# parsakhaz/multimodal-image-similarity-search

Hardware: AMD Instinct MI355X
Metric: images/s CLIP-B/32 encode @ bs256; Mvec/s cosine top-10 over 10M x 512 (higher is better)
Workload: dtype bf16

## Files before the change

### multimodal-image-similarity-search_amd/csrc/api_index.hip

```cpp
#include "common.h"
#include <queue>
#include "retrieval_kernels.h"
#include "gemm_bf16_256.h"
#include "gemm_bf16_p256.h"
#include <algorithm>

struct mmiss_index {
    int dim = 0, dtype = MMISS_F32, device = 0, elt = 4;
    int qelt() const { return dtype == MMISS_F32 ? 4 : 2; }
    hipStream_t own_stream = nullptr, user_stream = nullptr;
    bool has_user_stream = false;
    hipEvent_t done_ev = nullptr;
    bool async_pending = false;
    std::mutex mu;
    int64_t count = 0, capacity = 0;
    DevBuf rows, labels_d;
    DevBuf inv;
    std::vector<int64_t> labels_h;
    DevBuf tags;
    std::vector<uint64_t> tags_h;
    DevBuf fmask, fmask2, tag_stage;
    DevBuf stage, qn, qs, qstage, lists_s, lists_r, lists2_s, lists2_r, cand, cur_s, cur_r, out_c, map, gmax;
    DevBuf qmap, qmap64, qs2, cand2;
    DevBuf eps_q, thr, thr2, swp_cnt, swp_list;
// ... 511 lines not shown
    MM_NO_PENDING(ix, "mmiss_index_get_tags");
    std::vector<int64_t> lab;
    MM_TRY(fetch_i64(labels, n, lab));
    std::vector<uint64_t> val((size_t)n);
    for (int64_t i = 0; i < n; ++i) {
        const int64_t r = find_row(ix, lab[i]);
        if (r < 0) MM_FAIL(MMISS_ERR_ARG, "mmiss_index_get_tags: label %lld not in the index", (long long)lab[i]);
        val[i] = ix->tags_h[(size_t)r];
    }
    if (mmiss_is_device_ptr(out)) {
        MM_TRY(mmiss_use_device(ix->device));
        MM_HIP(hipMemcpyAsync(out, val.data(), (size_t)n * 8, hipMemcpyHostToDevice, ix->stream()));
        MM_HIP(hipStreamSynchronize(ix->stream()));
    } else {
        memcpy(out, val.data(), (size_t)n * 8);
    }
    return MMISS_OK;
}

namespace {

constexpr int SWEEP_CAP = 8192;

void guard_terms(const mmiss_index* ix, double* fixed, double* cnorm) {
    const double D = ix->dim;
    const double cn = ix->dtype == MMISS_F8 ? 1.07 : 1.0 + ldexp(1.0, -9);
    double e = 4.0 * D * ldexp(1.0, -24) * cn * (1.0 + ldexp(1.0, -9));
    if (ix->dtype != MMISS_F32) e += D * ldexp(1.0, -25) * cn;
    if (ix->dtype == MMISS_F8) e += ldexp(1.0, -23);
    *fixed = e * 1.003 + ldexp(1.0, -21);
    *cnorm = ix->dtype == MMISS_F32 ? 0.0 : cn * 1.003;
}

int launch_rerank(mmiss_index* ix, hipStream_t st, const RerankArgs& r, int blocks) {
    int npow = 1;
    while (npow < r.ncand) npow <<= 1;
    const int lds = npow * 8 + 16;
    MM_PROF("rerank", st, 2.0 * blocks * r.ncand * r.D, (double)blocks * r.ncand * r.D * ix->elt);
    const int threads = r.ncand >= 16 ? 1024 : 256;
    void (*kern)(RerankArgs) = with_storage(ix->dtype, [](auto s) { return &rerank_kernel<typename decltype(s)::T>; });
    if (lds > 32768) MM_TRY(mmiss_ensure_dyn_lds(reinterpret_cast<const void*>(kern), lds));
    hipLaunchKernelGGL(kern, dim3(blocks), dim3(threads), lds, st, r);
    MM_HIP(hipGetLastError());
    return MMISS_OK;
}

int exhaustive_queries(mmiss_index* ix, hipStream_t st, const mmiss_index::Pending& pd, const std::vector<int32_t>& which) {
    const int64_t N = ix->count;
    const int D = ix->dim, KP = 32;
    const int kk = (int)std::min<int64_t>(pd.k, N);
    const int kkpad = (int)round_up(std::max(kk, 1), KP);
    const int nq = (int)which.size();
    if (nq == 0 || N <= 0) return MMISS_OK;
    MM_TRY(ix->dist_all.ensure((size_t)N * 4));
    MM_TRY(ix->dist_pin.ensure((size_t)N * 4, st));
    const float* dist = ix->dist_pin.as<float>();
    std::vector<int32_t> cand((size_t)nq * kkpad, -1);
    typedef std::pair<float, int32_t> Ent;
    for (int i = 0; i < nq; ++i) {
        const int32_t q = which[i];
        {
            MM_PROF("canonical_scan", st, 2.0 * N * D, (double)N * D * ix->elt);
            const int grid = (int)std::min<int64_t>(8192, (N + 15) / 16);
            with_storage(ix->dtype, [&](auto s) {
                hipLaunchKernelGGL(canonical_scan_kernel<typename decltype(s)::T>, dim3(grid), dim3(256), 0, st, ix->rows.p, N, D,
                                   ix->qn.as<float>() + (size_t)q * D, ix->dist_all.as<float>(), (const float*)ix->inv.as<float>());
            });
// ... 265 lines not shown
    MM_TRY(ix->eps_q.ensure((size_t)Qpad * 4));
    MM_TRY(ix->thr.ensure((size_t)Qpad * 4));
    MM_PROF("prep_queries", st, 4.0 * Q * D, (double)Q * D * (8 + ix->elt));
    double eps_fixed, cnorm;
    guard_terms(ix, &eps_fixed, &cnorm);
    with_storage(ix->dtype, [&](auto s) {
        using QT = typename decltype(s)::Q;
        hipLaunchKernelGGL(prep_queries_kernel<QT>, dim3((Qpad + 3) / 4), dim3(256), 0, st, qsrc, ix->qn.as<float>(), ix->qs.as<QT>(),
                           Q, Qpad, D, ix->eps_q.as<float>(), eps_fixed, cnorm);
    });
    MM_HIP(hipGetLastError());
    return MMISS_OK;
}

int dense_pass(mmiss_index* ix, hipStream_t st, const QueryPlan& p, int Q) {
    const int D = ix->dim, kp = p.kp;
    const int64_t N = ix->count;
    const int ng = (int)(p.Ndense / 16);
    MM_TRY(ix->gmax.ensure((size_t)p.Mq * ng * 4));
    GemmEpi ep{};
    ep.out = ix->gmax.p; ep.ldo = ng; ep.m_valid = Q; ep.p0 = (int)N; ep.m_fast = 1;
    ep.aux = ix->inv.as<float>();
    {
        MM_PROF(p.dense8 ? (p.sample ? "score_gemm_f8_sample" : "score_gemm_f8") : (p.sample ? "score_gemm_f16_sample" : "score_gemm_f16"), st,
                2.0 * Q * (double)std::min<int64_t>(N, p.Ndense) * D, (double)std::min<int64_t>(N, p.Ndense) * D * ix->elt);
        if (p.big) MM_TRY(launch_strip_gemm(ix, st, p.strip_v3, ix->qs.p, ep, p.Mq, (int)p.Ndense, p.strip, nullptr));
        else MM_TRY((launch_gemm_inst<_Float16, 128, MMISS_EPI_GROUPMAX_F32>(st, ix->qs.p, ix->rows.p, ep, p.Mq, (int)p.Npad, D)));
    }
    const int units = (ng + 1023) / 1024;
    int splits = (1024 + Q - 1) / Q;
    if (splits > units) splits = units;
    if (splits > 32) splits = 32;
    if (splits < 1) splits = 1;
    MM_TRY(ix->lists_s.ensure((size_t)splits * Q * kp * 4));
    MM_TRY(ix->lists_r.ensure((size_t)splits * Q * kp * 4));
    SelectArgs sa{};
    sa.G = ix->gmax.as<float>(); sa.ldg = ng; sa.ng = ng; sa.kp = kp; sa.Q = Q;
    sa.out_s = ix->lists_s.as<float>(); sa.out_r = ix->lists_r.as<int32_t>();
    {
        MM_PROF("select_topk", st, 0.0, (double)Q * ng * 4);
        hipLaunchKernelGGL(select_topk_kernel, dim3(Q, splits), dim3(256), 0, st, sa);
        MM_HIP(hipGetLastError());
    }
    MergeArgs m{};
    m.in_s = ix->lists_s.as<float>(); m.in_r = ix->lists_r.as<int32_t>();
    m.L = splits; m.Q = Q; m.kp = kp;
    if (p.sample) {
        const int cap = p.filter_cap;
        MM_TRY(ix->seed_s.ensure((size_t)p.Mq * kp * 4));
        MM_TRY(ix->seed_r.ensure((size_t)p.Mq * kp * 4));
        MM_TRY(ix->fcnt.ensure((size_t)p.Mq * 4));
        MM_TRY(ix->fbuf_s.ensure((size_t)p.Mq * cap * 4));
        MM_TRY(ix->fbuf_g.ensure((size_t)p.Mq * cap * 4));
        {
            MergeArgs m1 = m;
            m1.lists_per_block = splits; m1.out_s = ix->seed_s.as<float>(); m1.out_r = ix->seed_r.as<int32_t>();
            MM_PROF("merge_lists", st, 0.0, (double)splits * Q * kp * 8);
            hipLaunchKernelGGL(merge_lists_kernel, dim3(Q, 1), dim3(256), 0, st, m1);
            MM_HIP(hipGetLastError());
        }
        MM_HIP(hipMemsetAsync(ix->fcnt.p, 0, (size_t)p.Mq * 4, st));
        StripFilter flt{};
        flt.tau = ix->seed_s.as<float>() + (kp - 1); flt.tau_stride = kp;
        flt.cnt = ix->fcnt.as<int32_t>(); flt.buf_s = ix->fbuf_s.as<float>(); flt.buf_g = ix->fbuf_g.as<int32_t>();
        flt.cap = cap; flt.bn_begin = (int)p.ns_tiles;
        {
            MM_PROF(p.dense8 ? "score_gemm_f8" : "score_gemm_f16", st, 2.0 * Q * (double)(N - p.Ndense) * D, (double)(N - p.Ndense) * D * ix->elt);
            MM_TRY(launch_strip_gemm(ix, st, p.strip_v3, ix->qs.p, ep, p.Mq, (int)p.Npad, p.strip, &flt));
        }
        m.in_s = ix->seed_s.as<float>(); m.in_r = ix->seed_r.as<int32_t>(); m.L = 1;
        m.flat_s = ix->fbuf_s.as<float>(); m.flat_r = ix->fbuf_g.as<int32_t>(); m.flat_cnt = ix->fcnt.as<int32_t>();
        m.flat_cap = cap;
    }
    m.cand = ix->cand.as<int32_t>(); m.cand_stride = p.ncand; m.page_off = 0;
    m.cur_s = ix->cur_s.as<float>(); m.cur_r = ix->cur_r.as<int32_t>();
    return launch_merge(ix, st, m);
}

int scan_pass(mmiss_index* ix, hipStream_t st, const QueryPlan& qp, int Q) {
    const mmiss_index::Pending& pd = ix->pend;
    const int kp = qp.kp;
    const ScanPlan p = plan_scan(ix->dim, ix->qelt(), Q, kp, ix->count);
    MM_TRY(ix->lists_s.ensure((size_t)p.slabs * Q * kp * 4));
    MM_TRY(ix->lists_r.ensure((size_t)p.slabs * Q * kp * 4));
    const bool paging = qp.pages > 1;
    if (paging) {
        std::vector<float> inf((size_t)Q, INFINITY);
        std::vector<int32_t> neg((size_t)Q, -1);
        MM_HIP(hipMemcpyAsync(ix->cur_s.p, inf.data(), (size_t)Q * 4, hipMemcpyHostToDevice, st));
        MM_HIP(hipMemcpyAsync(ix->cur_r.p, neg.data(), (size_t)Q * 4, hipMemcpyHostToDevice, st));
        MM_HIP(hipStreamSynchronize(st));
    }
    for (int page = 0; page < qp.pages; ++page) {
        ScanArgs a{};
        a.rows = ix->rows.p; a.N = ix->count; a.D = ix->dim; a.inv = ix->inv.as<float>(); a.qs = ix->qs.p; a.Q = Q;
        a.cur_s = paging ? ix->cur_s.as<float>() : nullptr;
        a.cur_r = paging ? ix->cur_r.as<int32_t>() : nullptr;
        a.kp = kp; a.tiles_per_block = p.tiles_per_block;
        a.out_s = ix->lists_s.as<float>(); a.out_r = ix->lists_r.as<int32_t>();
        if (pd.filt) { a.tags = ix->tags.as<uint64_t>(); a.req = pd.d_mask; a.exc = pd.d_mask + Q; }
        MM_TRY(launch_scan(ix, st, a, p));
        MergeArgs m{};
        m.in_s = ix->lists_s.as<float>(); m.in_r = ix->lists_r.as<int32_t>();
        m.L = p.slabs; m.Q = Q; m.kp = kp;
        m.cand = ix->cand.as<int32_t>(); m.cand_stride = qp.ncand; m.page_off = page * kp;
        m.cur_s = ix->cur_s.as<float>(); m.cur_r = ix->cur_r.as<int32_t>();
        MM_TRY(launch_merge(ix, st, m));
    }
// ... 332 lines not shown
```

### multimodal-image-similarity-search_amd/csrc/retrieval_kernels.h

```cpp
#pragma once
#include "common.h"
#include "gemm_bf16.h"
#include <math.h>
#include <type_traits>

#define SCAN_NEG_INF (-INFINITY)
#define SCAN_ROW_NONE 0x7fffffff

__device__ __forceinline__ double wave_butterfly_sum(double v) {
#pragma unroll
    for (int o = 32; o > 0; o >>= 1) v = v + __shfl_xor(v, o);
    return v;
}

#define MMISS_F8_SCALE 128.0f
struct F8 {
    uint8_t b;
    F8() = default;
    __device__ explicit F8(float y) { b = (uint8_t)(__builtin_amdgcn_cvt_pk_fp8_f32(y * MMISS_F8_SCALE, 0.0f, 0, false) & 0xff); }
    __device__ explicit operator float() const { return __builtin_amdgcn_cvt_f32_fp8((int)b, 0) * (1.0f / MMISS_F8_SCALE); }
};
__device__ __forceinline__ void f8x4_values(uint32_t w, float (&v)[4]) {
    v[0] = __builtin_amdgcn_cvt_f32_fp8((int)w, 0) * (1.0f / MMISS_F8_SCALE);
    v[1] = __builtin_amdgcn_cvt_f32_fp8((int)w, 1) * (1.0f / MMISS_F8_SCALE);
// ... 442 lines not shown
            if (lane >= 32 && lane - 32 < cw) {
                s = cs_all[(w * NQ + ql) * CAP + lane - 32];
                r = cr_all[(w * NQ + ql) * CAP + lane - 32];
            }
            wave_sort64(s, r, lane);
        }
        if (lane < a.kp) {
            const size_t o = ((size_t)blockIdx.x * a.Q + q) * a.kp + lane;
            a.out_s[o] = s;
            a.out_r[o] = (r == SCAN_ROW_NONE) ? -1 : r;
        }
    }
}

struct SelectArgs {
    const float* G;
    int ldg;
    int ng;
    int kp;
    float* out_s;
    int32_t* out_r;
    int Q;
};

__device__ __forceinline__ void lane_list_insert(float& ls, int& lr, float xs, int xr, int lane) {
    const unsigned long long better = __ballot(ls > xs || (ls == xs && lr < xr));
    const int p = __popcll(better);
    const float us = __int_as_float(__builtin_amdgcn_update_dpp(__float_as_int(ls), __float_as_int(ls), 0x138, 0xF, 0xF, false));
    const int ur = __builtin_amdgcn_update_dpp(lr, lr, 0x138, 0xF, 0xF, false);
    if (lane > p) { ls = us; lr = ur; }
    else if (lane == p) { ls = xs; lr = xr; }
}

__global__ __launch_bounds__(256) void select_topk_kernel(SelectArgs a) {
    __shared__ float ms[4][32];
    __shared__ int mr[4][32];
    const int tid = threadIdx.x, lane = tid & 63, wave = tid >> 6;
    const int q = blockIdx.x;
    const int nsplit = gridDim.y;
    const int units = (a.ng + 1023) / 1024;
    const int upb = (units + nsplit - 1) / nsplit;
    const int c_begin = blockIdx.y * upb * 1024;
    int c_end = c_begin + upb * 1024;
    if (c_end > a.ng) c_end = a.ng;
    const float* row = a.G + (size_t)q * a.ldg;

    float ls = SCAN_NEG_INF;
    int lr = SCAN_ROW_NONE;
    float tau = SCAN_NEG_INF;
    int tau_r = SCAN_ROW_NONE;
    auto fetch = [&](int c0) {
        const int c = c0 + lane * 4;
        f32x4 v = {SCAN_NEG_INF, SCAN_NEG_INF, SCAN_NEG_INF, SCAN_NEG_INF};
        if (c0 >= c_end) return v;
        if (c + 3 < c_end) {
            v = *reinterpret_cast<const f32x4*>(row + c);
        } else {
#pragma unroll
            for (int e = 0; e < 4; ++e)
                if (c + e < c_end) v[e] = row[c + e];
        }
        return v;
    };
    f32x4 vnext = fetch(c_begin + wave * 256);
    for (int c0 = c_begin + wave * 256; c0 < c_end; c0 += 1024) {
        const int c = c0 + lane * 4;
        const f32x4 v = vnext;
        vnext = fetch(c0 + 1024);
        const bool seed = (c0 == c_begin + wave * 256);
        if (seed) {
            ls = v[0];
            lr = (c < c_end) ? c : SCAN_ROW_NONE;
            wave_sort64(ls, lr, lane);
            tau = __shfl(ls, a.kp - 1);
            tau_r = __shfl(lr, a.kp - 1);
        }
#pragma unroll
        for (int e = 0; e < 4; ++e) {
            if (seed && e == 0) continue;
            const float s = v[e];
            unsigned long long m = __ballot(s > tau || (s == tau && c + e < tau_r));
            while (m) {
                const int src = __ffsll((long long)m) - 1;
                m &= m - 1;
                const float xs = __shfl(s, src);
                const int xr = c0 + src * 4 + e;
                if (!(xs > tau || (xs == tau && xr < tau_r))) continue;
                lane_list_insert(ls, lr, xs, xr, lane);
                tau = __shfl(ls, a.kp - 1);
                tau_r = __shfl(lr, a.kp - 1);
            }
        }
    }
    if (lane < 32) { ms[wave][lane] = ls; mr[wave][lane] = lr; }
    __syncthreads();
    if (wave == 0) {
        float s = (lane < 32) ? ms[0][lane] : ms[1][lane - 32];
        int r = (lane < 32) ? mr[0][lane] : mr[1][lane - 32];
        wave_sort64(s, r, lane);
        for (int w = 2; w < 4; ++w) {
            if (lane >= 32) { s = ms[w][lane - 32]; r = mr[w][lane - 32]; }
            wave_sort64(s, r, lane);
        }
        if (lane < a.kp) {
            const size_t o = ((size_t)blockIdx.y * a.Q + q) * a.kp + lane;
            a.out_s[o] = s;
            a.out_r[o] = (r == SCAN_ROW_NONE) ? -1 : r;
        }
    }
}

struct MergeArgs {
    const float* in_s;
    const int32_t* in_r;
    int L, Q, kp;
    int32_t* cand;
    int cand_stride, page_off;
    float* cur_s;
    int32_t* cur_r;
    int lists_per_block;
    float* out_s;
    int32_t* out_r;
    const float* flat_s;
    const int32_t* flat_r;
    const int32_t* flat_cnt;
    int flat_cap;
};

__global__ __launch_bounds__(256) void merge_lists_kernel(MergeArgs a) {
    __shared__ float cs[4][64];
    __shared__ int cr[4][64];
    __shared__ int cnt[4];
    const int tid = threadIdx.x, lane = tid & 63, wave = tid >> 6;
    const int q = blockIdx.x;
    const int kp = a.kp;
    if (lane == 0) cnt[wave] = 0;
    __builtin_amdgcn_fence(__ATOMIC_SEQ_CST, "wavefront");
    float tau = SCAN_NEG_INF;
    const int l_begin = a.out_s ? blockIdx.y * a.lists_per_block : 0;
    int l_end = a.out_s ? l_begin + a.lists_per_block : a.L;
    if (l_end > a.L) l_end = a.L;
    const int64_t list_total = (int64_t)(l_end > l_begin ? l_end - l_begin : 0) * kp;
    int64_t total = list_total;
    if (a.flat_s) {
        const int c = a.flat_cnt[q];
        total += c < a.flat_cap ? c : a.flat_cap;
    }
    const int NL = 64 - kp;
    auto fetch = [&](int64_t e0, float& s, int& r) {
        s = SCAN_NEG_INF;
        r = -1;
        const int64_t e = e0 + lane;
        if (lane < NL && e < total) {
            if (e < list_total) {
                const int64_t l = l_begin + e / kp;
                const int slot = (int)(e % kp);
                const size_t o = ((size_t)l * a.Q + q) * kp + slot;
                s = a.in_s[o];
                r = a.in_r[o];
            } else {
                const size_t o = (size_t)q * a.flat_cap + (size_t)(e - list_total);
                s = a.flat_s[o];
                r = a.flat_r[o];
            }
        }
    };
    float s, sn;
    int r, rn;
    int64_t e0 = (int64_t)wave * NL;
    fetch(e0, s, r);
    while (e0 < total) {
        const int64_t e1 = e0 + 4 * (int64_t)NL;
        fetch(e1, sn, rn);
        if (r >= 0 && s > tau) {
            const int pos = atomicAdd(&cnt[wave], 1);
            cs[wave][pos] = s;
            cr[wave][pos] = r;
        }
        __builtin_amdgcn_fence(__ATOMIC_SEQ_CST, "wavefront");
        const int c = cnt[wave];
        if (c > kp) {
            float ss = SCAN_NEG_INF;
            int rr = SCAN_ROW_NONE;
            if (lane < c) { ss = cs[wave][lane]; rr = cr[wave][lane]; }
            wave_sort64(ss, rr, lane);
            if (lane < kp) { cs[wave][lane] = ss; cr[wave][lane] = rr; }
            tau = __shfl(ss, kp - 1);
            if (lane == 0) cnt[wave] = kp;
            __builtin_amdgcn_fence(__ATOMIC_SEQ_CST, "wavefront");
        }
        e0 = e1;
        s = sn;
// ... 4 lines not shown
        float s = SCAN_NEG_INF;
        int r = SCAN_ROW_NONE;
        const int c0 = cnt[0];
        if (lane < c0) { s = cs[0][lane]; r = cr[0][lane]; }
        wave_sort64(s, r, lane);
        for (int w = 1; w < 4; ++w) {
            const int cw = cnt[w];
            if (cw == 0) continue;
            if (lane >= kp) { s = SCAN_NEG_INF; r = SCAN_ROW_NONE; }
            if (lane >= 32 && lane - 32 < cw) { s = cs[w][lane - 32]; r = cr[w][lane - 32]; }
            wave_sort64(s, r, lane);
        }
        const bool valid = lane < kp && r != SCAN_ROW_NONE;
        if (a.out_s) {
            if (lane < kp) {
                const size_t o = ((size_t)blockIdx.y * a.Q + q) * kp + lane;
                a.out_s[o] = valid ? s : SCAN_NEG_INF;
                a.out_r[o] = valid ? r : -1;
            }
            return;
        }
        if (lane < kp) a.cand[(size_t)q * a.cand_stride + a.page_off + lane] = valid ? r : -1;
        if (a.cur_s) {
            const unsigned long long m = __ballot(valid);
            const int nvalid = __popcll(m);
            const float ls = __shfl(s, nvalid > 0 ? nvalid - 1 : 0);
            const int lr = __shfl(r, nvalid > 0 ? nvalid - 1 : 0);
            if (lane == 0) {
                if (nvalid == kp) { a.cur_s[q] = ls; a.cur_r[q] = lr; }
                else { a.cur_s[q] = SCAN_NEG_INF; a.cur_r[q] = SCAN_ROW_NONE; }
            }
        }
    }
}

struct RerankArgs {
    const void* rows; int D;
    const float* qn;
    const int32_t* cand;
    int cand_stride, ncand;
    int group_mode;
    int64_t nrows;
    const int64_t* labels;
    int k;
    int64_t* out_labels;
    float* out_dist;
    int32_t* out_count;
    const int32_t* qmap;
    int32_t* out_rows;
    const float* tau;
    double eps;
    int32_t* flags;
    int32_t* nflag;
    int force_flag;
    const int32_t* ovf_cnt;
    int ovf_cap;
    const float* eps_q;
    float* thr_out;
    const int32_t* cand_cnt;
    const int32_t* bmap;
    const float* inv;
    int32_t* cnt_host;
};

template <typename T>
__device__ __forceinline__ void canon_partial_dots(const T* rv, bool live, const float* qp, int D, double (&acc)[4]) {
    acc[0] = acc[1] = acc[2] = acc[3] = 0.0;
    typedef typename std::conditional<sizeof(T) == 1, uint32_t, typename std::conditional<sizeof(T) == 2, u32x2, f32x4>::type>::type piece_t;
    for (int d0 = 0; d0 < D; d0 += 512) {
        piece_t w[8];
        f32x4 qq[8];
#pragma unroll
        for (int u = 0; u < 8; ++u) {
            w[u] = piece_t{};
            qq[u] = f32x4{0.f, 0.f, 0.f, 0.f};
            if (d0 + 64 * u < D) {
                qq[u] = *reinterpret_cast<const f32x4*>(qp + d0 + 64 * u);
                if (live) w[u] = *reinterpret_cast<const piece_t*>(rv + d0 + 64 * u);
            }
        }
#pragma unroll
        for (int u = 0; u < 8; ++u) {
            if (d0 + 64 * u < D) {
                float rr[4];
                if constexpr (sizeof(T) == 1) {
                    f8x4_values(w[u], rr);
                } else if constexpr (sizeof(T) == 2) {
                    const _Float16* h = reinterpret_cast<const _Float16*>(&w[u]);
#pragma unroll
                    for (int j = 0; j < 4; ++j) rr[j] = (float)h[j];
                } else {
#pragma unroll
                    for (int j = 0; j < 4; ++j) rr[j] = w[u][j];
                }
#pragma unroll
                for (int j = 0; j < 4; ++j) acc[j] = acc[j] + (double)qq[u][j] * (double)rr[j];
            }
        }
    }
}

template <typename T>
__global__ __launch_bounds__(1024) void rerank_kernel(RerankArgs a) {
    extern __shared__ __attribute__((aligned(16))) char smem[];
    const int tid = threadIdx.x, lane = tid & 63, wave = tid >> 6;
    const int b = blockIdx.x;
    const int q = a.qmap ? a.qmap[b] : b;
    const int lb = a.bmap ? a.bmap[b] : b;
    int nc = a.ncand;
    if (a.cand_cnt) {
        const int cc = a.cand_cnt[lb];
        if (a.cnt_host && tid == 0) a.cnt_host[b] = cc;
        nc = cc < nc ? cc : nc;
    }
    int npow = 1;
    while (npow < nc) npow <<= 1;
    float* sd = reinterpret_cast<float*>(smem);
    int32_t* sr = reinterpret_cast<int32_t*>(smem + (size_t)npow * 4);
    const float* qv = a.qn + (size_t)q * a.D;
    const int nthreads = blockDim.x, nwaves = blockDim.x >> 6;
    for (int i = tid; i < npow; i += nthreads) { sd[i] = INFINITY; sr[i] = INT32_MAX; }
    __syncthreads();
    const int p16 = lane & 15, sub = lane >> 4;
    for (int c0 = wave * 4; c0 < nc; c0 += nwaves * 4) {
        const int c = c0 + sub;
        int64_t row = -1;
        if (c < nc) {
            if (a.group_mode) {
                const int g = a.cand[(size_t)lb * a.cand_stride + (c >> 4)];
                if (g >= 0) {
                    row = groupmax_row(g, c & 15);
                    if (row >= a.nrows) row = -1;
                }
            } else {
                row = a.cand[(size_t)lb * a.cand_stride + c];
            }
        }
        const bool live = row >= 0;
        const T* rv = reinterpret_cast<const T*>(a.rows) + (size_t)(live ? row : 0) * a.D + 4 * p16;
        const float* qp = qv + 4 * p16;
        double acc[4];
        canon_partial_dots<T>(rv, live, qp, a.D, acc);
#pragma unroll
        for (int o = 8; o > 0; o >>= 1) {
#pragma unroll
            for (int j = 0; j < 4; ++j) acc[j] = acc[j] + __shfl_xor(acc[j], o);
        }
        const double t0 = acc[0] + acc[2], t1 = acc[1] + acc[3];
        double dot = t0 + t1;
        if (p16 == 0 && row >= 0) {
            if constexpr (sizeof(T) == 1) dot = dot * (double)a.inv[row];
            sd[c] = (float)(1.0 - dot);
            sr[c] = (int32_t)row;
        }
    }
    __syncthreads();
    for (int k = 2; k <= npow; k <<= 1) {
        for (int j = k >> 1; j > 0; j >>= 1) {
            for (int i = tid; i < npow; i += nthreads) {
                const int p = i ^ j;
                if (p > i) {
                    const float di = sd[i], dp = sd[p];
                    const int32_t li = sr[i], lp = sr[p];
                    const bool up = (i & k) == 0;
                    const bool i_first = (di < dp) || (di == dp && li < lp) || (dp != dp && di == di);
                    const bool p_first = (dp < di) || (dp == di && lp < li) || (di != di && dp == dp);
                    const bool swap = up ? p_first : i_first;
                    if (swap) { sd[i] = dp; sd[p] = di; sr[i] = lp; sr[p] = li; }
                }
            }
            __syncthreads();
        }
    }
    for (int i = tid; i < a.k; i += nthreads) {
        const bool ok = i < npow && sr[i] != INT32_MAX;
        a.out_labels[(size_t)q * a.k + i] = ok ? a.labels[sr[i]] : -1;
        a.out_dist[(size_t)q * a.k + i] = ok ? sd[i] : INFINITY;
    }
    const int64_t k_eff = (int64_t)a.k < a.nrows ? (int64_t)a.k : a.nrows;
    if (a.out_rows) {
        for (int i = tid; i < a.cand_stride && i < (int)((k_eff + 31) & ~31LL); i += nthreads)
            a.out_rows[(size_t)b * a.cand_stride + i] = (i < k_eff && i < npow && sr[i] != INT32_MAX) ? sr[i] : -1;
    }
    if (tid == 0) {
        int nvalid = 0;
        const int lim = a.k < npow ? a.k : npow;
        for (int i = 0; i < lim; ++i) nvalid += (sr[i] != INT32_MAX);
        a.out_count[q] = nvalid;
        const double eps = a.eps_q ? (double)a.eps_q[q] : a.eps;
        if (a.flags) {
            int flag = 0;
            const float t = a.tau ? a.tau[b] : SCAN_NEG_INF;
            if (t > SCAN_NEG_INF) {
                if (nvalid < k_eff || a.force_flag) flag = 1;
                else if (a.ovf_cnt && a.ovf_cnt[q] > a.ovf_cap) flag = 1;
                else {
                    const double ck = 1.0 - (double)sd[k_eff - 1];
                    if (!(ck - (double)t > eps)) flag = 1;
                }
            }
            a.flags[b] = flag;
            if (flag && a.nflag) atomicAdd(a.nflag, 1);
        }
        if (a.thr_out) {
            float thr = SCAN_NEG_INF;
            if (k_eff > 0 && nvalid >= k_eff) {
                const double lim = (1.0 - (double)sd[k_eff - 1]) - eps;
                thr = (float)lim;
                if ((double)thr > lim) thr = nextafterf(thr, -INFINITY);
                if (!(lim == lim)) thr = SCAN_NEG_INF;
            }
            a.thr_out[q] = thr;
        }
    }
}

template <typename T>
__global__ __launch_bounds__(256) void canonical_scan_kernel(const void* __restrict__ rows, int64_t N, int D,
                                                             const float* __restrict__ qv, float* __restrict__ dist,
                                                             const float* __restrict__ inv) {
    const int lane = threadIdx.x & 63, wave = threadIdx.x >> 6;
    const int p16 = lane & 15, sub = lane >> 4;
    const float* qp = qv + 4 * p16;
    for (int64_t r0 = ((int64_t)blockIdx.x * 4 + wave) * 4; r0 < N; r0 += (int64_t)gridDim.x * 16) {
        const int64_t row = r0 + sub;
        const bool live = row < N;
        const T* rv = reinterpret_cast<const T*>(rows) + (size_t)(live ? row : 0) * D + 4 * p16;
        double acc[4];
        canon_partial_dots<T>(rv, live, qp, D, acc);
#pragma unroll
        for (int o = 8; o > 0; o >>= 1) {
#pragma unroll
            for (int j = 0; j < 4; ++j) acc[j] = acc[j] + __shfl_xor(acc[j], o);
        }
        const double t0 = acc[0] + acc[2], t1 = acc[1] + acc[3];
        double dot = t0 + t1;
        if (p16 == 0 && live) {
            if constexpr (sizeof(T) == 1) dot = dot * (double)inv[row];
            dist[row] = (float)(1.0 - dot);
        }
// ... 132 lines not shown
```

### multimodal-image-similarity-search_amd/csrc/encoder_kernels.h

```cpp
#pragma once
#include "common.h"
#include "attention_stream.h"

template <bool SRC_U8>
__global__ __launch_bounds__(256) void im2col_kernel(const void* __restrict__ pixels, uint16_t* __restrict__ out,
                                                     int B, int S, int P, int Kp) {
    const int G = S / P;
    const int PP = P * P;
    const int Kreal = 3 * PP;
    const int kgroups = Kp >> 3;
    const int64_t total = (int64_t)B * G * G * kgroups;
    const float mean[3] = {0.48145466f, 0.4578275f, 0.40821073f};
    const float istd[3] = {1.0f / 0.26862954f, 1.0f / 0.26130258f, 1.0f / 0.27577711f};
    for (int64_t idx = (int64_t)blockIdx.x * blockDim.x + threadIdx.x; idx < total;
         idx += (int64_t)gridDim.x * blockDim.x) {
        const int kg = (int)(idx % kgroups);
        const int64_t m = idx / kgroups;
        const int b = (int)(m / (G * G));
        const int pr = (int)(m - (int64_t)b * G * G);
        const int py = pr / G, px = pr - py * G;
        const int k0 = kg << 3;
        float v[8];
        if (!SRC_U8 && (P & 7) == 0 && k0 < Kreal) {
            const int c = k0 / PP, rem = k0 - c * PP, ky = rem / P, kx = rem - ky * P;
            const float* src = reinterpret_cast<const float*>(pixels) +
                               (((size_t)b * 3 + c) * S + (size_t)py * P + ky) * S + (size_t)px * P + kx;
            const f32x4 a = *reinterpret_cast<const f32x4*>(src);
            const f32x4 d = *reinterpret_cast<const f32x4*>(src + 4);
            v[0] = a[0]; v[1] = a[1]; v[2] = a[2]; v[3] = a[3];
            v[4] = d[0]; v[5] = d[1]; v[6] = d[2]; v[7] = d[3];
        } else {
#pragma unroll
            for (int e = 0; e < 8; ++e) {
                const int k = k0 + e;
                float x = 0.f;
// ... 964 lines not shown
        case 6: return heads(std::integral_constant<int, 6>{});
    }
    const int lds = NKP * 32 * (128 + ATT_VSTRIDE);
    const int rounds = ((T + 15) / 16 + 3) / 4;
    int qs = 256 / (B * H);
    qs = qs < 1 ? 1 : (qs > rounds ? rounds : qs);
    MM_TRY(mmiss_ensure_dyn_lds(reinterpret_cast<const void*>(&attention_kernel<NKP, false, true>), lds));
    hipLaunchKernelGGL((attention_kernel<NKP, false, true>), dim3(B * H, qs), dim3(256), lds, st, (const uint16_t*)qkv, (uint16_t*)nullptr, T, H,
                       ctx8, ctxs, ld_s);
    MM_HIP(hipGetLastError());
    return MMISS_OK;
}
static int launch_attention_mx_short(hipStream_t st, const void* qkv, uint8_t* ctx8, uint8_t* ctxs, int ld_s, int B, int T, int H) {
    int hpb = mmiss_option("att_hpb", 0);
    if (hpb == 0) {
        hpb = 1;
        for (int c : {4, 6, 3, 2})
            if (H % c == 0 && (int64_t)B * (H / c) >= 512) { hpb = c; break; }
    }
    if (!((hpb == 2 || hpb == 3 || hpb == 4 || hpb == 6) && H % hpb == 0)) hpb = 1;
    switch ((T + 31) / 32) {
        case 1: return launch_attention_mx_nkp<1>(st, hpb, qkv, ctx8, ctxs, ld_s, B, T, H);
        case 2: return launch_attention_mx_nkp<2>(st, hpb, qkv, ctx8, ctxs, ld_s, B, T, H);
        case 3: return launch_attention_mx_nkp<3>(st, hpb, qkv, ctx8, ctxs, ld_s, B, T, H);
        default: return launch_attention_mx_nkp<4>(st, hpb, qkv, ctx8, ctxs, ld_s, B, T, H);
    }
}

static int launch_attention(hipStream_t st, const void* qkv, void* ctx, int B, int T, int H, bool causal) {
    if (B <= 0) return MMISS_OK;
    if (T <= 0 || T > 288 || H <= 0) MM_FAIL(MMISS_ERR_UNSUPPORTED, "attention: T=%d (1..288), H=%d", T, H);
    const int nkp = (T + 31) / 32;
    MM_PROF("attention", st, 4.0 * B * H * (double)T * T * 64, (double)B * T * H * 64 * 2 * 4);
    if (nkp <= 4) {
        int hpb = mmiss_option("att_hpb", 0);
        if (hpb == 0) {
            hpb = 1;
            for (int c : {4, 6, 3, 2})
                if (H % c == 0 && (int64_t)B * (H / c) >= 512) { hpb = c; break; }
        }
        if ((hpb == 2 || hpb == 3 || hpb == 4 || hpb == 6) && H % hpb == 0) {
            switch (nkp) {
                case 1: return launch_attention_heads_hpb<1>(st, hpb, qkv, ctx, B, T, H, causal);
                case 2: return launch_attention_heads_hpb<2>(st, hpb, qkv, ctx, B, T, H, causal);
                case 3: return launch_attention_heads_hpb<3>(st, hpb, qkv, ctx, B, T, H, causal);
                default: return launch_attention_heads_hpb<4>(st, hpb, qkv, ctx, B, T, H, causal);
            }
        }
    }
    switch (nkp) {
        case 1: return launch_attention_nkp<1>(st, qkv, ctx, B, T, H, causal);
        case 2: return launch_attention_nkp<2>(st, qkv, ctx, B, T, H, causal);
        case 3: return launch_attention_nkp<3>(st, qkv, ctx, B, T, H, causal);
        case 4: return launch_attention_nkp<4>(st, qkv, ctx, B, T, H, causal);
    }
    return causal ? launch_attention_long<true, false>(st, qkv, ctx, nullptr, nullptr, 0, B, T, H)
                  : launch_attention_long<false, false>(st, qkv, ctx, nullptr, nullptr, 0, B, T, H);
}
```

Measured before the change: 87540.

## Fuse top-k select and merge kernels; replace rerank bitonic sort with rank counting

For the non-sampled dense path, the per-split top-k select and the list merge now run in one kernel per query. Split lists are kept in shared memory, which removes a launch and a global round trip of the intermediate lists. In rerank, the full bitonic sort is replaced by direct rank computation (O(n^2) comparisons, no barriers) when the candidate count is at most 1024 and no NaN is present; the bitonic sort stays available behind an option. Wave shuffles with uniform source lanes become readlane. The fused kernel serialises splits within one block, which may lower parallelism when there are few queries.

```diff
diff --git a/multimodal-image-similarity-search_amd/csrc/api_index.hip b/multimodal-image-similarity-search_amd/csrc/api_index.hip
--- a/multimodal-image-similarity-search_amd/csrc/api_index.hip
+++ b/multimodal-image-similarity-search_amd/csrc/api_index.hip
@@ -567,7 +567,8 @@
     *cnorm = ix->dtype == MMISS_F32 ? 0.0 : cn * 1.003;
 }
 
-int launch_rerank(mmiss_index* ix, hipStream_t st, const RerankArgs& r, int blocks) {
+int launch_rerank(mmiss_index* ix, hipStream_t st, RerankArgs r, int blocks) {
+    r.bitonic = mmiss_option("rerank_bitonic", 0);
     int npow = 1;
     while (npow < r.ncand) npow <<= 1;
     const int lds = npow * 8 + 16;
@@ -899,19 +900,27 @@
     if (splits > units) splits = units;
     if (splits > 32) splits = 32;
     if (splits < 1) splits = 1;
+    SelectArgs sa{};
+    sa.G = ix->gmax.as<float>(); sa.ldg = ng; sa.ng = ng; sa.kp = kp; sa.Q = Q;
+    MergeArgs m{};
+    m.L = splits; m.Q = Q; m.kp = kp;
+    m.cand = ix->cand.as<int32_t>(); m.cand_stride = p.ncand; m.page_off = 0;
+    m.cur_s = ix->cur_s.as<float>(); m.cur_r = ix->cur_r.as<int32_t>();
+    if (!p.sample && mmiss_option("select_fused", 1) != 0) {
+        MM_PROF("select_merge", st, 0.0, (double)Q * ng * 4);
+        hipLaunchKernelGGL(select_merge_kernel, dim3(Q), dim3(256 * std::min(splits, 4)), 0, st, sa, m);
+        MM_HIP(hipGetLastError());
+        return MMISS_OK;
+    }
     MM_TRY(ix->lists_s.ensure((size_t)splits * Q * kp * 4));
     MM_TRY(ix->lists_r.ensure((size_t)splits * Q * kp * 4));
-    SelectArgs sa{};
-    sa.G = ix->gmax.as<float>(); sa.ldg = ng; sa.ng = ng; sa.kp = kp; sa.Q = Q;
     sa.out_s = ix->lists_s.as<float>(); sa.out_r = ix->lists_r.as<int32_t>();
     {
         MM_PROF("select_topk", st, 0.0, (double)Q * ng * 4);
         hipLaunchKernelGGL(select_topk_kernel, dim3(Q, splits), dim3(256), 0, st, sa);
         MM_HIP(hipGetLastError());
     }
-    MergeArgs m{};
     m.in_s = ix->lists_s.as<float>(); m.in_r = ix->lists_r.as<int32_t>();
-    m.L = splits; m.Q = Q; m.kp = kp;
     if (p.sample) {
         const int cap = p.filter_cap;
         MM_TRY(ix->seed_s.ensure((size_t)p.Mq * kp * 4));
@@ -939,8 +948,6 @@
         m.flat_s = ix->fbuf_s.as<float>(); m.flat_r = ix->fbuf_g.as<int32_t>(); m.flat_cnt = ix->fcnt.as<int32_t>();
         m.flat_cap = cap;
     }
-    m.cand = ix->cand.as<int32_t>(); m.cand_stride = p.ncand; m.page_off = 0;
-    m.cur_s = ix->cur_s.as<float>(); m.cur_r = ix->cur_r.as<int32_t>();
     return launch_merge(ix, st, m);
 }
 
diff --git a/multimodal-image-similarity-search_amd/csrc/retrieval_kernels.h b/multimodal-image-similarity-search_amd/csrc/retrieval_kernels.h
--- a/multimodal-image-similarity-search_amd/csrc/retrieval_kernels.h
+++ b/multimodal-image-similarity-search_amd/csrc/retrieval_kernels.h
@@ -498,21 +498,18 @@
     else if (lane == p) { ls = xs; lr = xr; }
 }
 
-__global__ __launch_bounds__(256) void select_topk_kernel(SelectArgs a) {
-    __shared__ float ms[4][32];
-    __shared__ int mr[4][32];
-    const int tid = threadIdx.x, lane = tid & 63, wave = tid >> 6;
-    const int q = blockIdx.x;
-    const int nsplit = gridDim.y;
-    const int units = (a.ng + 1023) / 1024;
+__device__ __forceinline__ void select_range(int ng, int nsplit, int y, int& c_begin, int& c_end) {
+    const int units = (ng + 1023) / 1024;
     const int upb = (units + nsplit - 1) / nsplit;
-    const int c_begin = blockIdx.y * upb * 1024;
-    int c_end = c_begin + upb * 1024;
-    if (c_end > a.ng) c_end = a.ng;
-    const float* row = a.G + (size_t)q * a.ldg;
-
-    float ls = SCAN_NEG_INF;
-    int lr = SCAN_ROW_NONE;
+    c_begin = y * upb * 1024;
+    c_end = c_begin + upb * 1024;
+    if (c_end > ng) c_end = ng;
+}
+
+__device__ __forceinline__ void select_wave_list(const float* row, int c_begin, int c_end, int kp, int wave, int lane, float& ls,
+                                                 int& lr) {
+    ls = SCAN_NEG_INF;
+    lr = SCAN_ROW_NONE;
     float tau = SCAN_NEG_INF;
     int tau_r = SCAN_ROW_NONE;
     auto fetch = [&](int c0) {
@@ -538,8 +535,8 @@
             ls = v[0];
             lr = (c < c_end) ? c : SCAN_ROW_NONE;
             wave_sort64(ls, lr, lane);
-            tau = __shfl(ls, a.kp - 1);
-            tau_r = __shfl(lr, a.kp - 1);
+            tau = __int_as_float(__builtin_amdgcn_readlane(__float_as_int(ls), kp - 1));
+            tau_r = __builtin_amdgcn_readlane(lr, kp - 1);
         }
 #pragma unroll
         for (int e = 0; e < 4; ++e) {
@@ -549,25 +546,43 @@
             while (m) {
                 const int src = __ffsll((long long)m) - 1;
                 m &= m - 1;
-                const float xs = __shfl(s, src);
+                const float xs = __int_as_float(__builtin_amdgcn_readlane(__float_as_int(s), src));
                 const int xr = c0 + src * 4 + e;
                 if (!(xs > tau || (xs == tau && xr < tau_r))) continue;
                 lane_list_insert(ls, lr, xs, xr, lane);
-                tau = __shfl(ls, a.kp - 1);
-                tau_r = __shfl(lr, a.kp - 1);
-            }
-        }
-    }
+                tau = __int_as_float(__builtin_amdgcn_readlane(__float_as_int(ls), kp - 1));
+                tau_r = __builtin_amdgcn_readlane(lr, kp - 1);
+            }
+        }
+    }
+}
+
+__device__ __forceinline__ void select_fold4(const float (*ms)[32], const int (*mr)[32], int lane, float& s, int& r) {
+    s = (lane < 32) ? ms[0][lane] : ms[1][lane - 32];
+    r = (lane < 32) ? mr[0][lane] : mr[1][lane - 32];
+    wave_sort64(s, r, lane);
+    for (int w = 2; w < 4; ++w) {
+        if (lane >= 32) { s = ms[w][lane - 32]; r = mr[w][lane - 32]; }
+        wave_sort64(s, r, lane);
+    }
+}
+
+__global__ __launch_bounds__(256) void select_topk_kernel(SelectArgs a) {
+    __shared__ float ms[4][32];
+    __shared__ int mr[4][32];
+    const int tid = threadIdx.x, lane = tid & 63, wave = tid >> 6;
+    const int q = blockIdx.x;
+    int c_begin, c_end;
+    select_range(a.ng, gridDim.y, blockIdx.y, c_begin, c_end);
+    float ls;
+    int lr;
+    select_wave_list(a.G + (size_t)q * a.ldg, c_begin, c_end, a.kp, wave, lane, ls, lr);
     if (lane < 32) { ms[wave][lane] = ls; mr[wave][lane] = lr; }
     __syncthreads();
     if (wave == 0) {
-        float s = (lane < 32) ? ms[0][lane] : ms[1][lane - 32];
-        int r = (lane < 32) ? mr[0][lane] : mr[1][lane - 32];
-        wave_sort64(s, r, lane);
-        for (int w = 2; w < 4; ++w) {
-            if (lane >= 32) { s = ms[w][lane - 32]; r = mr[w][lane - 32]; }
-            wave_sort64(s, r, lane);
-        }
+        float s;
+        int r;
+        select_fold4(ms, mr, lane, s, r);
         if (lane < a.kp) {
             const size_t o = ((size_t)blockIdx.y * a.Q + q) * a.kp + lane;
             a.out_s[o] = s;
@@ -593,14 +608,14 @@
     int flat_cap;
 };
 
-__global__ __launch_bounds__(256) void merge_lists_kernel(MergeArgs a) {
+template <typename ListEntry>
+__device__ __forceinline__ void merge_lists_block(const MergeArgs& a, int q, bool active, ListEntry list) {
     __shared__ float cs[4][64];
     __shared__ int cr[4][64];
     __shared__ int cnt[4];
     const int tid = threadIdx.x, lane = tid & 63, wave = tid >> 6;
-    const int q = blockIdx.x;
     const int kp = a.kp;
-    if (lane == 0) cnt[wave] = 0;
+    if (active && lane == 0) cnt[wave] = 0;
     __builtin_amdgcn_fence(__ATOMIC_SEQ_CST, "wavefront");
     float tau = SCAN_NEG_INF;
     const int l_begin = a.out_s ? blockIdx.y * a.lists_per_block : 0;
@@ -612,6 +627,7 @@
         const int c = a.flat_cnt[q];
         total += c < a.flat_cap ? c : a.flat_cap;
     }
+    if (!active) total = 0;
     const int NL = 64 - kp;
     auto fetch = [&](int64_t e0, float& s, int& r) {
         s = SCAN_NEG_INF;
@@ -619,11 +635,7 @@
         const int64_t e = e0 + lane;
         if (lane < NL && e < total) {
             if (e < list_total) {
-                const int64_t l = l_begin + e / kp;
-                const int slot = (int)(e % kp);
-                const size_t o = ((size_t)l * a.Q + q) * kp + slot;
-                s = a.in_s[o];
-                r = a.in_r[o];
+                list(l_begin + e / kp, (int)(e % kp), s, r);
             } else {
                 const size_t o = (size_t)q * a.flat_cap + (size_t)(e - list_total);
                 s = a.flat_s[o];
@@ -694,6 +706,52 @@
             }
         }
     }
+}
+
+__global__ __launch_bounds__(256) void merge_lists_kernel(MergeArgs a) {
+    const int q = blockIdx.x;
+    merge_lists_block(a, q, true, [&](int64_t l, int slot, float& s, int& r) {
+        const size_t o = ((size_t)l * a.Q + q) * a.kp + slot;
+        s = a.in_s[o];
+        r = a.in_r[o];
+    });
+}
+
+__global__ __launch_bounds__(1024) void select_merge_kernel(SelectArgs a, MergeArgs m) {
+    __shared__ float ms[4][4][32];
+    __shared__ int mr[4][4][32];
+    __shared__ float lst_s[32 * 32];
+    __shared__ int lst_r[32 * 32];
+    const int tid = threadIdx.x, lane = tid & 63, wave = tid >> 6;
+    const int grp = wave >> 2, gw = wave & 3, groups = blockDim.x >> 8;
+    const int q = blockIdx.x, S = m.L, kp = a.kp;
+    const float* row = a.G + (size_t)q * a.ldg;
+    for (int y0 = 0; y0 < S; y0 += groups) {
+        const int y = y0 + grp;
+        float ls = SCAN_NEG_INF;
+        int lr = SCAN_ROW_NONE;
+        if (y < S) {
+            int c_begin, c_end;
+            select_range(a.ng, S, y, c_begin, c_end);
+            select_wave_list(row, c_begin, c_end, kp, gw, lane, ls, lr);
+        }
+        if (lane < 32) { ms[grp][gw][lane] = ls; mr[grp][gw][lane] = lr; }
+        __syncthreads();
+        if (y < S && gw == 0) {
+            float s;
+            int r;
+            select_fold4(ms[grp], mr[grp], lane, s, r);
+            if (lane < kp) {
+                lst_s[y * kp + lane] = s;
+                lst_r[y * kp + lane] = (r == SCAN_ROW_NONE) ? -1 : r;
+            }
+        }
+        __syncthreads();
+    }
+    merge_lists_block(m, q, wave < 4, [&](int64_t l, int slot, float& s, int& r) {
+        s = lst_s[l * kp + slot];
+        r = lst_r[l * kp + slot];
+    });
 }
 
 struct RerankArgs {
@@ -723,6 +781,7 @@
     const int32_t* bmap;
     const float* inv;
     int32_t* cnt_host;
+    int bitonic;
 };
 
 template <typename T>
@@ -762,13 +821,24 @@
     }
 }
 
+#define RERANK_RANK_MAX 1024
+
 template <typename T>
 __global__ __launch_bounds__(1024) void rerank_kernel(RerankArgs a) {
     extern __shared__ __attribute__((aligned(16))) char smem[];
+    __shared__ int nreal_s;
+    __shared__ float kth_s;
     const int tid = threadIdx.x, lane = tid & 63, wave = tid >> 6;
     const int b = blockIdx.x;
     const int q = a.qmap ? a.qmap[b] : b;
     const int lb = a.bmap ? a.bmap[b] : b;
+    float g_tau = SCAN_NEG_INF, g_eps = 0.f;
+    int g_ovf = 0;
+    if (tid == 0) {
+        if (a.tau) g_tau = a.tau[b];
+        if (a.eps_q) g_eps = a.eps_q[q];
+        if (a.ovf_cnt) g_ovf = a.ovf_cnt[q];
+    }
     int nc = a.ncand;
     if (a.cand_cnt) {
         const int cc = a.cand_cnt[lb];
@@ -782,8 +852,11 @@
     const float* qv = a.qn + (size_t)q * a.D;
     const int nthreads = blockDim.x, nwaves = blockDim.x >> 6;
     for (int i = tid; i < npow; i += nthreads) { sd[i] = INFINITY; sr[i] = INT32_MAX; }
+    if (tid == 0) nreal_s = 0;
     __syncthreads();
     const int p16 = lane & 15, sub = lane >> 4;
+    int nlive = 0;
+    bool nan_d = false;
     for (int c0 = wave * 4; c0 < nc; c0 += nwaves * 4) {
         const int c = c0 + sub;
         int64_t row = -1;
@@ -810,55 +883,96 @@
         }
         const double t0 = acc[0] + acc[2], t1 = acc[1] + acc[3];
         double dot = t0 + t1;
+        nlive += __popcll(__ballot(p16 == 0 && live));
         if (p16 == 0 && row >= 0) {
             if constexpr (sizeof(T) == 1) dot = dot * (double)a.inv[row];
-            sd[c] = (float)(1.0 - dot);
+            const float d = (float)(1.0 - dot);
+            sd[c] = d;
             sr[c] = (int32_t)row;
-        }
-    }
-    __syncthreads();
-    for (int k = 2; k <= npow; k <<= 1) {
-        for (int j = k >> 1; j > 0; j >>= 1) {
-            for (int i = tid; i < npow; i += nthreads) {
-                const int p = i ^ j;
-                if (p > i) {
-                    const float di = sd[i], dp = sd[p];
-                    const int32_t li = sr[i], lp = sr[p];
-                    const bool up = (i & k) == 0;
-                    const bool i_first = (di < dp) || (di == dp && li < lp) || (dp != dp && di == di);
-                    const bool p_first = (dp < di) || (dp == di && lp < li) || (di != di && dp == dp);
-                    const bool swap = up ? p_first : i_first;
-                    if (swap) { sd[i] = dp; sd[p] = di; sr[i] = lp; sr[p] = li; }
+            nan_d |= d != d;
+        }
+    }
+    if (lane == 0 && nlive) atomicAdd(&nreal_s, nlive);
+    const bool any_nan = __syncthreads_or(nan_d) != 0;
+    const int nreal = nreal_s;
+    const int64_t k_eff = (int64_t)a.k < a.nrows ? (int64_t)a.k : a.nrows;
+    const int out_rows_n = (int)((k_eff + 31) & ~31LL);
+    if (!a.bitonic && !any_nan && nc <= RERANK_RANK_MAX) {
+        for (int c = tid; c < nc; c += nthreads) {
+            const int32_t r = sr[c];
+            if (r == INT32_MAX) continue;
+            const float d = sd[c];
+            int rk = 0;
+            for (int j = 0; j < nc; ++j) {
+                const float dj = sd[j];
+                const int32_t rj = sr[j];
+                rk += (dj < d) || (dj == d && (rj < r || (rj == r && j < c)));
+            }
+            if (rk < a.k) {
+                a.out_labels[(size_t)q * a.k + rk] = a.labels[r];
+                a.out_dist[(size_t)q * a.k + rk] = d;
+            }
+            if (a.out_rows && rk < k_eff && rk < a.cand_stride) a.out_rows[(size_t)b * a.cand_stride + rk] = r;
+            if (rk == k_eff - 1) kth_s = d;
+        }
+        for (int i = nreal + tid; i < a.k; i += nthreads) {
+            a.out_labels[(size_t)q * a.k + i] = -1;
+            a.out_dist[(size_t)q * a.k + i] = INFINITY;
+        }
+        if (a.out_rows) {
+            const int i0 = (int64_t)nreal < k_eff ? nreal : (int)k_eff;
+            for (int i = i0 + tid; i < a.cand_stride && i < out_rows_n; i += nthreads) a.out_rows[(size_t)b * a.cand_stride + i] = -1;
+        }
+        __syncthreads();
+    } else {
+        for (int k = 2; k <= npow; k <<= 1) {
+            for (int j = k >> 1; j > 0; j >>= 1) {
+                for (int i = tid; i < npow; i += nthreads) {
+                    const int p = i ^ j;
+                    if (p > i) {
+                        const float di = sd[i], dp = sd[p];
+                        const int32_t li = sr[i], lp = sr[p];
+                        const bool up = (i & k) == 0;
+                        const bool i_first = (di < dp) || (di == dp && li < lp) || (dp != dp && di == di);
+                        const bool p_first = (dp < di) || (dp == di && lp < li) || (di != di && dp == dp);
+                        const bool swap = up ? p_first : i_first;
+                        if (swap) { sd[i] = dp; sd[p] = di; sr[i] = lp; sr[p] = li; }
+                    }
                 }
-            }
-            __syncthreads();
-        }
-    }
-    for (int i = tid; i < a.k; i += nthreads) {
-        const bool ok = i < npow && sr[i] != INT32_MAX;
-        a.out_labels[(size_t)q * a.k + i] = ok ? a.labels[sr[i]] : -1;
-        a.out_dist[(size_t)q * a.k + i] = ok ? sd[i] : INFINITY;
-    }
-    const int64_t k_eff = (int64_t)a.k < a.nrows ? (int64_t)a.k : a.nrows;
-    if (a.out_rows) {
-        for (int i = tid; i < a.cand_stride && i < (int)((k_eff + 31) & ~31LL); i += nthreads)
-            a.out_rows[(size_t)b * a.cand_stride + i] = (i < k_eff && i < npow && sr[i] != INT32_MAX) ? sr[i] : -1;
+                __syncthreads();
+            }
+        }
+        for (int i = tid; i < a.k; i += nthreads) {
+            const bool ok = i < npow && sr[i] != INT32_MAX;
+            a.out_labels[(size_t)q * a.k + i] = ok ? a.labels[sr[i]] : -1;
+            a.out_dist[(size_t)q * a.k + i] = ok ? sd[i] : INFINITY;
+        }
+        if (a.out_rows) {
+            for (int i = tid; i < a.cand_stride && i < out_rows_n; i += nthreads)
+                a.out_rows[(size_t)b * a.cand_stride + i] = (i < k_eff && i < npow && sr[i] != INT32_MAX) ? sr[i] : -1;
+        }
     }
     if (tid == 0) {
         int nvalid = 0;
         const int lim = a.k < npow ? a.k : npow;
-        for (int i = 0; i < lim; ++i) nvalid += (sr[i] != INT32_MAX);
+        float kth = 0.f;
+        if (!a.bitonic && !any_nan && nc <= RERANK_RANK_MAX) {
+            nvalid = nreal < lim ? nreal : lim;
+            kth = kth_s;
+        } else {
+            for (int i = 0; i < lim; ++i) nvalid += (sr[i] != INT32_MAX);
+            if (k_eff > 0 && nvalid >= k_eff) kth = sd[k_eff - 1];
+        }
         a.out_count[q] = nvalid;
-        const double eps = a.eps_q ? (double)a.eps_q[q] : a.eps;
+        const double eps = a.eps_q ? (double)g_eps : a.eps;
         if (a.flags) {
             int flag = 0;
-            const float t = a.tau ? a.tau[b] : SCAN_NEG_INF;
-            if (t > SCAN_NEG_INF) {
+            if (g_tau > SCAN_NEG_INF) {
                 if (nvalid < k_eff || a.force_flag) flag = 1;
-                else if (a.ovf_cnt && a.ovf_cnt[q] > a.ovf_cap) flag = 1;
+                else if (a.ovf_cnt && g_ovf > a.ovf_cap) flag = 1;
                 else {
-                    const double ck = 1.0 - (double)sd[k_eff - 1];
-                    if (!(ck - (double)t > eps)) flag = 1;
+                    const double ck = 1.0 - (double)kth;
+                    if (!(ck - (double)g_tau > eps)) flag = 1;
                 }
             }
             a.flags[b] = flag;
@@ -867,7 +981,7 @@
         if (a.thr_out) {
             float thr = SCAN_NEG_INF;
             if (k_eff > 0 && nvalid >= k_eff) {
-                const double lim = (1.0 - (double)sd[k_eff - 1]) - eps;
+                const double lim = (1.0 - (double)kth) - eps;
                 thr = (float)lim;
                 if ((double)thr > lim) thr = nextafterf(thr, -INFINITY);
                 if (!(lim == lim)) thr = SCAN_NEG_INF;
```

Measured after the change: 87300, median of 2. About the same (-0.3%).

## Add persistent triple-buffered DMA attention kernel for short non-causal sequences

Applied to the files above, without the earlier changes.

Adds a persistent attention kernel for T<=64 non-causal cases. Each workgroup walks a contiguous range of (batch, head) pairs and stages Q/K/V into a three-slot LDS ring with buffer-load-to-LDS DMA, so loading the next pairs overlaps the MFMA softmax-attention of the current one. The aim is to hide global-memory latency and launch/tail overhead of the per-head kernels for short sequences such as CLIP vision (T=50). It adds LDS pressure and relies on hand-written waitcnt and barrier sequencing, which could be fragile.

```diff
diff --git a/multimodal-image-similarity-search_amd/csrc/attention_short_stream.h b/multimodal-image-similarity-search_amd/csrc/attention_short_stream.h
--- /dev/null
+++ b/multimodal-image-similarity-search_amd/csrc/attention_short_stream.h
@@ -0,0 +1,161 @@
+#pragma once
+#include "attention_stream.h"
+
+#define ASS_SLOTS 3
+#define ASS_WGS 512
+
+template <int NKP>
+__device__ __forceinline__ void ass_tile(const char* sK, const char* sV, const bf16x8 (&qf)[2], int q, int T, int fr, int fg,
+                                         uint16_t* orow) {
+    f32x4 sacc[2 * NKP];
+    float mx = -INFINITY;
+#pragma unroll
+    for (int kt = 0; kt < 2 * NKP; ++kt) {
+        f32x4 a = {0.f, 0.f, 0.f, 0.f};
+        const int krow = kt * 16 + fr;
+#pragma unroll
+        for (int s = 0; s < 2; ++s) {
+            const int chunk = 4 * s + fg;
+            const bf16x8 kf = *reinterpret_cast<const bf16x8*>(sK + krow * 128 + ((chunk ^ (krow & 7)) << 4));
+            a = __builtin_amdgcn_mfma_f32_16x16x32_bf16(kf, qf[s], a, 0, 0, 0);
+        }
+#pragma unroll
+        for (int r = 0; r < 4; ++r) {
+            const int key = kt * 16 + 4 * fg + r;
+            a[r] = key < T ? a[r] * 0.125f : -INFINITY;
+            mx = fmaxf(mx, a[r]);
+        }
+        sacc[kt] = a;
+    }
+    mx = fmaxf(mx, __shfl_xor(mx, 16));
+    mx = fmaxf(mx, __shfl_xor(mx, 32));
+    float l = 0.f;
+#pragma unroll
+    for (int kt = 0; kt < 2 * NKP; ++kt)
+#pragma unroll
+        for (int r = 0; r < 4; ++r) {
+            const float pexp = __expf(sacc[kt][r] - mx);
+            sacc[kt][r] = pexp;
+            l += pexp;
+        }
+    l += __shfl_xor(l, 16);
+    l += __shfl_xor(l, 32);
+
+    f32x4 oacc[4];
+#pragma unroll
+    for (int dt = 0; dt < 4; ++dt) oacc[dt] = f32x4{0.f, 0.f, 0.f, 0.f};
+    const int tq = fr >> 2, tp = fr & 3;
+#pragma unroll
+    for (int ks = 0; ks < NKP; ++ks) {
+        u32x4 praw;
+        praw[0] = pack_bf16x2(sacc[2 * ks][0], sacc[2 * ks][1]);
+        praw[1] = pack_bf16x2(sacc[2 * ks][2], sacc[2 * ks][3]);
+        praw[2] = pack_bf16x2(sacc[2 * ks + 1][0], sacc[2 * ks + 1][1]);
+        praw[3] = pack_bf16x2(sacc[2 * ks + 1][2], sacc[2 * ks + 1][3]);
+        const bf16x8 pf = __builtin_bit_cast(bf16x8, praw);
+#pragma unroll
+        for (int dt = 0; dt < 4; ++dt) {
+            const int vrow = 32 * ks + 4 * fg + tq;
+            const char* a0 = sV + vrow * 128 + ((dt ^ ((vrow >> 1) & 3)) << 5) + 8 * tp;
+            const bf16x4 v0 = __builtin_amdgcn_ds_read_tr16_b64_v4bf16((__attribute__((address_space(3))) bf16x4*)(a0));
+            const bf16x4 v1 = __builtin_amdgcn_ds_read_tr16_b64_v4bf16((__attribute__((address_space(3))) bf16x4*)(a0 + 16 * 128));
+            bf16x8 vf;
+            vf[0] = v0[0]; vf[1] = v0[1]; vf[2] = v0[2]; vf[3] = v0[3];
+            vf[4] = v1[0]; vf[5] = v1[1]; vf[6] = v1[2]; vf[7] = v1[3];
+            oacc[dt] = __builtin_amdgcn_mfma_f32_16x16x32_bf16(vf, pf, oacc[dt], 0, 0, 0);
+        }
+    }
+    const float inv = 1.0f / l;
+    asm volatile("s_waitcnt vmcnt(%0)" ::"n"(3 * NKP) : "memory");
+    if (q < T) {
+#pragma unroll
+        for (int dt = 0; dt < 4; ++dt) {
+            u32x2 pk;
+            pk[0] = pack_bf16x2(oacc[dt][0] * inv, oacc[dt][1] * inv);
+            pk[1] = pack_bf16x2(oacc[dt][2] * inv, oacc[dt][3] * inv);
+            *reinterpret_cast<u32x2*>(orow + dt * 16) = pk;
+        }
+    }
+}
+
+template <int NKP>
+__global__ __launch_bounds__(256) void attention_short_stream_kernel(const uint16_t* __restrict__ qkv, uint16_t* __restrict__ ctx,
+                                                                     int T, int H, int npairs, int per) {
+    extern __shared__ __attribute__((aligned(16))) char smem[];
+    constexpr int TP = NKP * 32;
+    constexpr int OPB = TP * 128;
+    constexpr int SLOT = 3 * OPB;
+    constexpr int NPW = 3 * NKP;
+    const int tid = threadIdx.x, lane = tid & 63;
+    const int wave = __builtin_amdgcn_readfirstlane(tid >> 6);
+    const int fr = lane & 15, fg = lane >> 4;
+    const int dmodel = H * 64, ld2 = 6 * dmodel;
+    const uint32_t lds0 = (uint32_t)(uintptr_t)((__attribute__((address_space(3))) char*)smem);
+    const int first = blockIdx.x * per;
+    const int cnt = min(per, npairs - first);
+    const int prow = lane >> 3, cp = lane & 7;
+    const int qklane = prow * ld2 + ((cp ^ prow) << 4);
+    const int vlane = prow * ld2 + ((cp ^ (((prow >> 1) & 3) << 1)) << 4) + 4 * dmodel;
+
+    int sb = first / H, sh = first - sb * H;
+    int cb = sb, ch = sh;
+    auto stage = [&](bool live, int slot) {
+        const uint64_t a = (uint64_t)(qkv + (size_t)sb * T * 3 * dmodel);
+        const u32x4 srd = {(uint32_t)a, (uint32_t)(a >> 32) & 0xffffu, live ? (uint32_t)(T * ld2) : 0u, 0x00020000u};
+        const uint32_t img = lds0 + slot * SLOT;
+#pragma unroll
+        for (int i = 0; i < NPW; ++i) {
+            const int op = i / NKP, p = wave + 4 * (i % NKP);
+            ats_dma16(srd, img + op * OPB + p * 1024, (op == 2 ? vlane : qklane + op * 2 * dmodel) + p * 8 * ld2 + sh * 128);
+        }
+        if (live && ++sh == H) { sh = 0; ++sb; }
+    };
+    stage(true, 0);
+    stage(cnt > 1, 1);
+    if (T < TP) {
+        for (int i = tid; i < ASS_SLOTS * 3 * (TP - T) * 8; i += 256) {
+            const int r = i >> 3, im = r / (TP - T);
+            *reinterpret_cast<u32x4*>(smem + im * OPB + (T + r - im * (TP - T)) * 128 + (i & 7) * 16) = u32x4{0u, 0u, 0u, 0u};
+        }
+    }
+    asm volatile("s_waitcnt vmcnt(%0)\n\ts_waitcnt lgkmcnt(0)\n\ts_barrier" ::"n"(NPW) : "memory");
+
+    const int nqt = (T + 15) >> 4;
+    int cur = 0;
+#pragma unroll 1
+    for (int n = 0; n < cnt; ++n) {
+        stage(n + 2 < cnt, cur == 0 ? ASS_SLOTS - 1 : cur - 1);
+        const char* sQ = smem + cur * SLOT;
+        if (wave < nqt) {
+            const int q = wave * 16 + fr;
+            bf16x8 qf[2];
+#pragma unroll
+            for (int s = 0; s < 2; ++s) qf[s] = *reinterpret_cast<const bf16x8*>(sQ + q * 128 + (((4 * s + fg) ^ (q & 7)) << 4));
+            ass_tile<NKP>(sQ + OPB, sQ + 2 * OPB, qf, q, T, fr, fg, ctx + ((size_t)cb * T + q) * dmodel + ch * 64 + 4 * fg);
+        } else {
+            asm volatile("s_waitcnt vmcnt(%0)" ::"n"(NPW) : "memory");
+        }
+        asm volatile("s_waitcnt lgkmcnt(0)\n\ts_barrier" ::: "memory");
+        if (++ch == H) { ch = 0; ++cb; }
+        cur = cur == ASS_SLOTS - 1 ? 0 : cur + 1;
+    }
+    asm volatile("s_waitcnt vmcnt(0)" ::: "memory");
+}
+
+static inline bool attention_short_stream_ok(int B, int T, int H, bool causal) {
+    return !causal && T > 0 && T <= 64 && H > 0 && (int64_t)B * H >= mmiss_option("att_short_stream_min_pairs", 2 * ASS_WGS) &&
+           64ll * 6 * H * 64 < (1ll << 31);
+}
+
+template <int NKP>
+static int launch_attention_short_stream(hipStream_t st, const void* qkv, void* ctx, int B, int T, int H) {
+    const int npairs = B * H;
+    const int per = (npairs + ASS_WGS - 1) / ASS_WGS;
+    const int grid = (npairs + per - 1) / per;
+    const int lds = ASS_SLOTS * 3 * NKP * 32 * 128;
+    MM_TRY(mmiss_ensure_dyn_lds(reinterpret_cast<const void*>(&attention_short_stream_kernel<NKP>), lds));
+    hipLaunchKernelGGL((attention_short_stream_kernel<NKP>), dim3(grid), dim3(256), lds, st, (const uint16_t*)qkv, (uint16_t*)ctx, T,
+                       H, npairs, per);
+    MM_HIP(hipGetLastError());
+    return MMISS_OK;
+}
diff --git a/multimodal-image-similarity-search_amd/csrc/encoder_kernels.h b/multimodal-image-similarity-search_amd/csrc/encoder_kernels.h
--- a/multimodal-image-similarity-search_amd/csrc/encoder_kernels.h
+++ b/multimodal-image-similarity-search_amd/csrc/encoder_kernels.h
@@ -1,6 +1,7 @@
 #pragma once
 #include "common.h"
 #include "attention_stream.h"
+#include "attention_short_stream.h"
 
 template <bool SRC_U8>
 __global__ __launch_bounds__(256) void im2col_kernel(const void* __restrict__ pixels, uint16_t* __restrict__ out,
@@ -1031,6 +1032,8 @@
     if (T <= 0 || T > 288 || H <= 0) MM_FAIL(MMISS_ERR_UNSUPPORTED, "attention: T=%d (1..288), H=%d", T, H);
     const int nkp = (T + 31) / 32;
     MM_PROF("attention", st, 4.0 * B * H * (double)T * T * 64, (double)B * T * H * 64 * 2 * 4);
+    if (attention_short_stream_ok(B, T, H, causal) && mmiss_option("att_short_stream", 1))
+        return nkp == 1 ? launch_attention_short_stream<1>(st, qkv, ctx, B, T, H) : launch_attention_short_stream<2>(st, qkv, ctx, B, T, H);
     if (nkp <= 4) {
         int hpb = mmiss_option("att_hpb", 0);
         if (hpb == 0) {
```

New measurement: 87280 before, 86450 after (median of 2 runs). About the same (-0.9%).
